# cxy1997/3D_adapt_auto_driving

Hardware: AMD Instinct MI355X
Metric: KITTI scenes/s end-to-end eval_rcnn (joint RPN+RCNN, synthetic 16384-pt scenes) (higher is better)
Workload: dtype f32; 1 GPU; BASELINE.json configs[2]: full PointRCNN RPN+RCNN inference, default.yaml shapes, random-init weights, batch=8 synthetic KITTI scenes x 16384 pts per GPU per step; scene=synth.scenes (SURVEY 8d: uniform clutter + ground + 10 dense cars), parallelism=scene-sharded x1, one final all_gather of detections, detections_gathered=652455, batch_slots=14, look_ahead=12, steps_per_launch=2

## Files before the change

3d_adapt_auto_driving_amd/_lib.py:

```python
import ctypes as C
import os

_HERE = os.path.dirname(os.path.abspath(__file__))
LIB_PATH = os.path.join(_HERE, "lib", "libprcnn_hip.so")

_P = C.c_void_p
_I = C.c_int
_F = C.c_float
_D = C.c_double
_L = C.c_longlong

class GatherProblem(C.Structure):
    _fields_ = [("b", _I), ("n", _I), ("c1", _I), ("max_tiles", C.c_long), ("P", _P), ("wxyz", _P), ("rowinfo", _P), ("rowdxyz", _P),
                ("tilecloud", _P), ("hdr", _P), ("out", _P)]


class LayerProblem(C.Structure):
    _fields_ = [("hdr", _P), ("rows", C.c_long), ("max_tiles", C.c_long), ("K", _I), ("N", _I), ("n_store", _I), ("A", _P), ("lda", C.c_long),
                ("W", _P), ("bias", _P), ("relu", _I), ("out", _P), ("ldo", C.c_long), ("b", _I), ("m", _I), ("rowinfo", _P), ("tilecloud", _P),
                ("out_col", _I), ("out_is_zero", _I)]


class SaProblem(C.Structure):
    _fields_ = [("b", _I), ("n", _I), ("m", _I), ("c3", _I), ("max_tiles", C.c_long), ("P", _P), ("wxyz", _P), ("rowinfo", _P), ("rowdxyz", _P),
# ... 21 lines not shown
    "prcnn_three_interpolate": [_I, _I, _I, _I, _P, _P, _P, _P, _P],
    "prcnn_three_interpolate_grad": [_I, _I, _I, _I, _P, _P, _P, _P, _P],
    "prcnn_query_and_group": [_I, _I, _I, _I, _F, _I, _P, _P, _P, _P, _P, _P],
    "prcnn_bias_relu_inplace": [C.c_long, _I, C.c_long, _P, _P, _P],
    "prcnn_maxpool_bias_relu": [_I, _I, _I, _I, _P, _P, _P, _P],
    "prcnn_group_cat_pm": [_I, _I, _I, _I, _I, _P, _P, _P, _P, _P, _P],
    "prcnn_gather_affine_relu_pm": [_I, _I, _I, _I, _I, _P, _P, _P, _P, _P, _P, _P],
    "prcnn_sa_mlp_fused": [_I] * 7 + [_P] * 10 + [_I, _I, _P],
    "prcnn_ball_pack": [_I, _I, _I, _I, _P, _P, _P, _P, _P, _P, _P, _P, _P],
    "prcnn_ball_pack_ex": [_I, _I, _I, _I, _I, _P, _P, _P, _P, _P, _P, _P, _P, _P, _P, _I, _P],
    "prcnn_rcnn_postprocess_blobs": [_I, _I, _I, _F, _F, _I, _I, _F, _F, _P, _F, _F, _P, _P, _P, _P, _P, _I, _P],
    "prcnn_ball_pack_groups": [_I, _I, _I, _I, _I, _P, _P, _P, _P, _P, _P, _P, _P, _P],
    "prcnn_ball_pack_rep": [_I, _I, _I, _I, _P, _P, _P, _P, _P, _P, _P, _P, _P, _P, _P],
    "prcnn_dup_rep": [_I, _I, _I, _P, _P, _P, _P, _P],
    "prcnn_rcnn_roi_geometry": [_I, _I, _I, _F, _I, _I, _F, _I] + [_P] * 9,
    "prcnn_rcnn_roi_geometry_packs": [_I, _I, _I, _F, _I, _I, _F, _I] + [_P] * 21 + [_I, _P],
    "prcnn_rows_gemm128_rows": [_L, _P, _I, _I, _P, _P, _I, _P, _P, _P, _P],
    "prcnn_sa_packed_mlp": [_I, _I, _I, _I, C.c_long] + [_P] * 11 + [_I, _I, _I, _P],
    "prcnn_packed_gather_affine": [_I, _I, _I, C.c_long] + [_P] * 7 + [_P],
    "prcnn_packed_layer": [_P, C.c_long, C.c_long, _I, _I, _I, _P, C.c_long, _P, _P, _I, _P, C.c_long, _P],
    "prcnn_split_weights_bf16x3": [_I, _I, _P, _P, _P],
    "prcnn_rows_layer_bf16x3": [C.c_long, _I, _I, _I, _P, C.c_long, _P, _P, _I, _P, C.c_long, _P],
    "prcnn_packed_layer_interp": [C.c_long, _I, _I, _P, C.c_long, _P, _P, _I, _P, C.c_long, _I, _I, _P, C.c_long, _P, _P, _P],
    "prcnn_sa_xyz_mlp_packed": [_I, _I, _I, _I, _I, C.c_long] + [_P] * 11 + [_I, _I, _I, _P],
    "prcnn_rows_dot": [C.c_long, _I, _I, _P, C.c_long, _P, _P, _P, C.c_long, _P],
    "prcnn_sa_wide_fused_supported": [_I, _I, _I],
    "prcnn_sa_wide_fused": [_I, _I, _I, _I, _I, _I, C.c_long] + [_P] * 11 + [_I, _I, _I, _P],
    "prcnn_sa_wide_fused3_supported": [_I, _I, _I, _I],
    "prcnn_sa_wide_fused3": [_I, _I, _I, _I, _I, _I, _I, C.c_long] + [_P] * 11 + [_I, _I, _I, _P],
    "prcnn_sa_packed_mlp_batch": [_I, C.POINTER(SaProblem), _P],
    "prcnn_packed_gather_affine_batch": [_I, C.POINTER(GatherProblem), _P],
    "prcnn_packed_layer_batch": [_I, C.POINTER(LayerProblem), _I, _P],
    "prcnn_rpn_tail": [_I, _I, _I] + [_P] * 7 + [_I] + [_P] * 4,
    "prcnn_rpn_tail_lin": [_I, _I, _I] + [_P] * 7 + [_I] + [_P] * 4,
    "prcnn_rpn_tail_boxes_supported": [_I, _F, _F, _I, _I],
    "prcnn_rpn_tail_lin_boxes": [_I, _I, _I] + [_P] * 7 + [_I, _F, _F, _I, _I] + [_P] * 6,
    "prcnn_selftest_fmod_two_pi": [_L, _P, _P, _P, _P],
    "prcnn_rpn_proposals_boxes": [_I, _I, _I, _I, _F, _I, _P, _P, _P, _P, _P],
    "prcnn_packed_layer_segmax": [_I, _I, C.c_long, _I, _I, _P, C.c_long, _P, _P, _P, _P, _P, _P, _I, _I, _I, _P],
    "prcnn_maxpool_pm": [C.c_long, _I, _I, _P, _P, _I, _I, _P],
    "prcnn_three_interpolate_pm": [_I, _I, _I, _I, _P, _P, _P, _P, _I, _I, _P],
    "prcnn_three_interpolate_cat_pm": [_I, _I, _I, _I, _P, _P, _P, _P, _I, _P, _P],
    "prcnn_boxes_overlap_bev": [_I, _P, _I, _P, _P, _P],
    "prcnn_boxes_iou_bev": [_I, _P, _I, _P, _P, _P],
    "prcnn_nms": [_I, _P, _P, _F, _P],
    "prcnn_nms_normal": [_I, _P, _P, _F, _P],
# ... 101 lines not shown
```

3d_adapt_auto_driving_amd/dropin/pointnet2_cuda.py:

```python
import ctypes
import importlib
import os
import sys

import torch

_pkg_dir = os.path.dirname(os.path.dirname(os.path.abspath(__file__)))
if os.path.dirname(_pkg_dir) not in sys.path:
    sys.path.insert(0, os.path.dirname(_pkg_dir))
_lib = importlib.import_module(os.path.basename(_pkg_dir) + "._lib")
IS_HIP_EXTENSION = True


def _chk(dtype, *tensors):
    for t in tensors:
        if not t.is_cuda:
            raise RuntimeError("pointnet2_cuda: tensor must be a CUDA tensor")
        if not t.is_contiguous():
            raise RuntimeError("pointnet2_cuda: tensor must be contiguous")
        if t.dtype != dtype:
            raise RuntimeError("pointnet2_cuda: expected %s, got %s" % (dtype, t.dtype))


def ball_query_wrapper(b, n, m, radius, nsample, new_xyz, xyz, idx):
# ... 441 lines not shown
        _SPLIT_W[key] = ws
    _lib.call("prcnn_rows_layer_bf16x3", R, K, N, out.size(1), a.data_ptr(), a.stride(0), ws.data_ptr(), bias.data_ptr(), int(bool(relu)),
              out.data_ptr(), out.stride(0), _lib.current_stream(a))
    return out


def packed_layer_interp_wrapper(a, wt, bias, relu, out, G, idx, weight):
    _chk(torch.float32, wt, bias, G, weight)
    _chk(torch.int32, idx)
    for t in (a, out):
        if not t.is_cuda or t.dtype != torch.float32 or t.dim() != 2 or t.stride(1) != 1:
            raise RuntimeError("pointnet2_cuda: packed_layer_interp expects 2-D float32 CUDA matrices with unit column stride")
    R, K = a.shape
    N = wt.size(1)
    B, n = idx.shape[0], idx.shape[1]
    if wt.size(0) != K or tuple(out.shape) != (R, N) or R != B * n or G.shape[0] != B or G.shape[2] != N or tuple(weight.shape) != tuple(idx.shape):
        raise RuntimeError("pointnet2_cuda: packed_layer_interp shape mismatch")
    _lib.call("prcnn_packed_layer_interp", R, K, N, a.data_ptr(), a.stride(0), wt.data_ptr(), bias.data_ptr(), int(bool(relu)),
              out.data_ptr(), out.stride(0), n, G.shape[1], G.data_ptr(), G.stride(1), idx.data_ptr(), weight.data_ptr(),
              _lib.current_stream(a))
    return out


def sa_wide_fused_supported(c1, c2, c3):
    return bool(_lib.load().prcnn_sa_wide_fused_supported(int(c1), int(c2), int(c3)))


def sa_wide_fused_wrapper(new_xyz, xyz, P, wxyz, pack, w2t, b2, w3t, b3, out, out_col, zeroed=False):
    _chk(torch.float32, new_xyz, xyz, P, wxyz, w2t, b2, w3t, b3, out)
    b, n, c1 = P.shape
    if w2t.size(0) != c1 or w3t.size(0) != w2t.size(1) or wxyz.size(1) != c1:
        raise RuntimeError("pointnet2_cuda: sa_wide_fused shape mismatch")
    _lib.call("prcnn_sa_wide_fused", b, n, new_xyz.size(1), c1, w2t.size(1), w3t.size(1), pack.max_tiles, P.data_ptr(), wxyz.data_ptr(),
              pack.rowinfo.data_ptr(), pack.rowdxyz.data_ptr(), pack.tilecloud.data_ptr(), pack.hdr.data_ptr(), w2t.data_ptr(),
              b2.data_ptr(), w3t.data_ptr(), b3.data_ptr(), out.data_ptr(), out.size(-1), out_col, int(bool(zeroed)),
              _lib.current_stream(xyz))
    return out


def sa_wide_fused3_supported(c0, c1, c2, c3):
    return bool(_lib.load().prcnn_sa_wide_fused3_supported(int(c0), int(c1), int(c2), int(c3)))


def sa_wide_fused3_wrapper(new_xyz, xyz, feats, wcat, b1, wxyz, pack, b2, b3, widths, out, out_col, zeroed=False):
    _chk(torch.float32, new_xyz, xyz, feats, wcat, b1, wxyz, b2, b3, out)
    b, n, c0 = feats.shape
# ... 213 lines not shown
```

3d_adapt_auto_driving_amd/net/fast_infer.py:

```python
import os

import torch

from ..pointnet2 import pointnet2_utils as pu
from ..pointnet2 import fused_mlp
from .._lib import has_entry
from .. import kitti_utils
from .. import roipool3d_utils
from .. import iou3d_utils


USE_ROIPOOL_CANONICAL = True
USE_RCNN_POINT_MLP = True
USE_XYZ_MLP = True
USE_PACKED = os.environ.get("PRCNN_NO_PACK") is None
USE_POOL_DEDUP = os.environ.get("PRCNN_NO_POOL_DEDUP") is None
USE_POINT_LAYER = os.environ.get("PRCNN_LIB_GEMM") is None
PAD128 = USE_PACKED and USE_POINT_LAYER
USE_RPN_TAIL = os.environ.get("PRCNN_NO_RPN_TAIL") is None
USE_SCALE_BATCH = True
USE_SA_NARROW = True
USE_WIDE_FUSED = True
EARLY_LEVELS = int(os.environ.get("PRCNN_EARLY_LEVELS", "4"))
EARLY_FP = int(os.environ.get("PRCNN_EARLY_FP", "2"))
# ... 86 lines not shown
                           % (wt.shape[0], wt.shape[1], a.shape[0]))
    if relu:
        try:
            return torch._addmm_activation(bias, a, wt)
        except (AttributeError, RuntimeError):
            return torch.addmm(bias, a, wt).relu_()
    return torch.addmm(bias, a, wt)


SPLIT_BF16 = os.environ.get("PRCNN_SPLIT_BF16") == "1"


def point_layer(a, wt, bias, relu, n_out=None):
    K, N = wt.shape
    n_out = N if n_out is None else n_out
    if (USE_PACKED and K % 128 == 0 and N % 128 == 0 and a.dim() == 2 and a.shape[1] == K and a.stride(1) == 1
            and a.stride(0) % 4 == 0 and a.data_ptr() % 16 == 0):
        out = torch.empty((a.shape[0], n_out), dtype=torch.float32, device=a.device)
        if SPLIT_BF16 and getattr(pu.pointnet2, "IS_HIP_EXTENSION", False):
            return pu.pointnet2.rows_layer_bf16x3_wrapper(a, wt, bias, relu, out)
        return pu.pointnet2.packed_layer_wrapper(a, wt, bias, relu, out)
    y = gemm_bias_act(a, wt, bias, relu)
    return y if n_out == N else y[:, :n_out].contiguous()


class _Mlp:

    def __init__(self, layers, grouped_c=None, pad128=False, in_parts=None, pad_out=False):
        self.layers = []
        self.n_out = layers[-1][0].shape[0]
        if pad128 and grouped_c is None:
            for i, (w, b, relu) in enumerate(layers):
                np_ = _round128(w.shape[0])
                if i == 0 and in_parts:
                    assert sum(in_parts) == w.shape[1]
                    wt = w.new_zeros((sum(_round128(c) for c in in_parts), np_))
                    src = dst = 0
                    for c in in_parts:
                        wt[dst:dst + c, :w.shape[0]] = w[:, src:src + c].t()
                        src, dst = src + c, dst + _round128(c)
                else:
                    wt = _pad2(w.t(), _round128(w.shape[1]), np_)
                self.layers.append((wt.contiguous(), _pad1(b, np_), relu))
            self.split = self.packed = self.wide = self.wide_cat = None
            self.padded = not pad_out
            self.narrow = None
# ... 309 lines not shown
        if not (USE_PACKED and USE_XYZ_MLP and self.sa and self.sa[0][1] and
                all(sc[3] == 0 for sc in self.sa[0][1])):
            return
        l_xyz, prev = geo["l_xyz"], None
        B = l_xyz[0].shape[0]
        for k in range(min(EARLY_LEVELS, len(self.sa))):
            npoint, scales = self.sa[k]
            lev = geo["sa"][k]
            packs = lev.get("pack") or [None] * len(scales)
            pre = bool(all(sc[2].packed is not None or sc[2].wide is not None or sc[3] == 0 for sc in scales))
            if not pre or any(pk is None for pk in packs):
                return
            width = sum(sc[2].layers[-1][0].shape[1] for sc in scales)
            oshape = (B, npoint, _round128(width) if PAD128 else width)
            out = arena.take(oshape) if arena is not None else torch.zeros(oshape, dtype=torch.float32, device=l_xyz[0].device)
            self._sa_level(scales, lev, l_xyz[k], prev, out, True)
            lev["out"] = prev = out
        if EARLY_FP > 0 and all(lev.get("out") is not None for lev in geo["sa"]) and len(geo["sa"]) == len(self.sa):
            l_feat = [None] + [lev["out"] for lev in geo["sa"]]
            geo["fp_out"] = {}
            for i in range(-1, -(min(EARLY_FP, len(self.fp) - 1) + 1), -1):
                kk = len(self.fp) + i
                idx, weight = geo["fp"][kk]
                l_feat[kk] = geo["fp_out"][kk] = self._fp_module(kk, l_feat[kk + 1], l_feat[kk], idx, weight)

    @staticmethod
    def _sa_scale(xyz, new_xyz, feats, idx, mlp, cin, out, out_col, P_pre=None, pack=None, zeroed=False, dense=False):
        ext = pu.pointnet2
        B, N, _ = xyz.shape
        M, ns = idx.shape[1], idx.shape[2]
        if USE_PACKED and mlp.packed is not None:
            wf, wx, b1, w2, b2, w3, b3 = mlp.packed
            P = P_pre if P_pre is not None else point_layer(feats.view(B * N, feats.shape[2]), wf, b1, False).view(B, N, 128)
            pk = pack if pack is not None else ext.ball_pack_wrapper(idx, xyz, new_xyz)
            ext.sa_packed_mlp_wrapper(new_xyz, xyz, P, wx, pk, w2, b2, w3, b3, out, out_col, zeroed)
            return
        if USE_PACKED and mlp.wide is not None:
            wf, wx, b1, w2, b2, w3, b3 = mlp.wide
            pk = pack if pack is not None else ext.ball_pack_wrapper(idx, xyz, new_xyz)
            if (dense and USE_WIDE_FUSED and has_entry(ext, "sa_wide_fused3_wrapper") and feats.is_contiguous() and
                    feats.shape[2] == wf.shape[0] and ext.sa_wide_fused3_supported(wf.shape[0], wf.shape[1], w2.shape[1], w3.shape[1])):
                ext.sa_wide_fused3_wrapper(new_xyz, xyz, feats, mlp.wide_cat, b1, wx, pk, b2, b3,
                                           (wf.shape[0], wf.shape[1], w2.shape[1], w3.shape[1]), out, out_col, zeroed)
                return
            P = point_layer(feats.view(B * N, feats.shape[2]), wf, b1, False).view(B, N, -1)
            if (dense and USE_WIDE_FUSED and has_entry(ext, "sa_wide_fused_wrapper") and
                    ext.sa_wide_fused_supported(wf.shape[1], w2.shape[1], w3.shape[1])):
# ... 75 lines not shown
                m0 = scales[0][2]
                if getattr(m0, "_pcat", None) is None or m0._pcat[2] is not scales[1][2].packed[0]:
                    m0._pcat = (torch.cat([sc[2].packed[0][:, :64] for sc in scales], 1).contiguous(),
                                torch.cat([sc[2].packed[2][:64] for sc in scales]).contiguous(), scales[1][2].packed[0])
                Pcat = torch.empty((B * N, 128), dtype=torch.float32, device=cur_xyz.device)
                ext.packed_layer_wrapper(flat, m0._pcat[0], m0._pcat[1], False, Pcat)
                Ps = [Pcat.view(B, N, 128)[:, :, 64 * k:64 * k + 64] for k in range(2)]
            else:
                Ps = [torch.empty((B * N, 128), dtype=torch.float32, device=cur_xyz.device) for _ in scales]
                ext.packed_layer_batch_wrapper([(flat, sc[2].packed[0], sc[2].packed[2], False, P, None) for sc, P in zip(scales, Ps)])
                Ps = [P.view(B, N, 128) for P in Ps]
            probs, col = [], 0
            for (radius, ns, mlp, cin), pack, P in zip(scales, packs, Ps):
                wf, wx, b1, w2, b2, w3, b3 = mlp.packed
                probs.append((lev["new_xyz"], cur_xyz, P, wx, pack, w2, b2, w3, b3, out, col, pre, mlp.packed_widths))
                col += mlp.layers[-1][0].shape[1]
            ext.sa_packed_mlp_batch_wrapper(probs)
        else:
            col = 0
            for (radius, ns, mlp, cin), idx, pack in zip(scales, lev["idx"], packs):
                self._sa_scale(cur_xyz, lev["new_xyz"], cur_feat, idx, mlp, cin, out, col, pack=pack, zeroed=pre)
                col += mlp.layers[-1][0].shape[1]

    def _backbone(self, xyz, geo, fuse_tail=False, feats0=None):
        l_xyz, l_feat = geo["l_xyz"], [feats0]
        B = xyz.shape[0]
        shapes, pres = [], []
        for npoint, scales in self.sa:
            width = sum(s[2].layers[-1][0].shape[1] for s in scales)
            shapes.append((B, npoint, _round128(width) if PAD128 else width))
            pres.append(bool(USE_PACKED and all(sc[2].packed is not None or sc[2].wide is not None or sc[3] == 0 for sc in scales)))
        early = [lev.get("out") if (lev.get("out") is not None and tuple(lev["out"].shape) == sh) else None for lev, sh in zip(geo["sa"], shapes)]
        sizes = [sh[0] * sh[1] * sh[2] if (pr and e is None) else 0 for sh, pr, e in zip(shapes, pres, early)]
        arena = torch.zeros((sum(sizes),), dtype=torch.float32, device=xyz.device) if sum(sizes) else None
        offs = [sum(sizes[:k]) for k in range(len(sizes))]
        for k, ((npoint, scales), lev) in enumerate(zip(self.sa, geo["sa"])):
            if early[k] is not None:
                l_feat.append(early[k])
                continue
            cur_xyz, cur_feat = l_xyz[len(l_feat) - 1], l_feat[-1]
            width = sum(s[2].layers[-1][0].shape[1] for s in scales)
            wpad = shapes[k][2]
            pre = pres[k]
            out = (arena[offs[k]:offs[k] + sizes[k]].view(shapes[k]) if pre
                   else torch.empty(shapes[k], dtype=torch.float32, device=xyz.device))
            if wpad > width and not pre:
                out[:, :, width:] = 0
            self._sa_level(scales, lev, cur_xyz, cur_feat, out, pre)
            l_feat.append(out)
        ext = pu.pointnet2
        for i in range(-1, -(len(self.fp) + 1), -1):
            k = len(self.fp) + i
            if geo.get("fp_out", {}).get(k) is not None:
                l_feat[k] = geo["fp_out"][k]
                continue
            known_feat, skip = l_feat[k + 1], l_feat[k]
            idx, weight = geo["fp"][k]
            if fuse_tail and k == 0 and self.rpn_tail is not None and skip is None and known_feat.shape[2] == 256:
                return None, (known_feat, idx, weight)
            l_feat[k] = self._fp_module(k, known_feat, skip, idx, weight)
        return (l_feat[0], None) if fuse_tail else l_feat[0]

    def _fp_module(self, k, known_feat, skip, idx, weight):
        ext = pu.pointnet2
        B, n = idx.shape[0], idx.shape[1]
        c2 = known_feat.shape[2]
        c1 = 0 if skip is None else skip.shape[2]
        mlp = self.fp[k]
        wt, b1, relu1 = mlp.layers[0]
        if (USE_FP_LINEAR and USE_POINT_LAYER and PAD128 and c1 and c1 % 128 == 0 and c2 % 128 == 0 and wt.shape[0] == c2 + c1
                and wt.shape[1] % 128 == 0 and len(mlp.layers) >= 2 and has_entry(ext, "packed_layer_interp_wrapper")):
            m = known_feat.shape[1]
            N1 = wt.shape[1]
            if getattr(self, "_zero_bias", None) is None or self._zero_bias.numel() < N1 or self._zero_bias.device != wt.device:
                self._zero_bias = torch.zeros((max(N1, 1024),), dtype=torch.float32, device=wt.device)
            G = point_layer(known_feat.view(B * m, c2), wt[:c2], self._zero_bias[:N1], False).view(B, m, N1)
            y1 = torch.empty((B * n, N1), dtype=torch.float32, device=known_feat.device)
            ext.packed_layer_interp_wrapper(skip.view(B * n, c1), wt[c2:], b1, relu1, y1, G, idx, weight)
            return mlp(y1, start=1).view(B, n, -1)
        buf = torch.empty((B, n, c2 + c1), dtype=torch.float32, device=known_feat.device)
        if c1 and c1 % 4 == 0 and c2 % 4 == 0 and has_entry(ext, "three_interpolate_cat_pm_wrapper"):
            ext.three_interpolate_cat_pm_wrapper(known_feat, idx, weight, skip, buf)
        else:
            ext.three_interpolate_pm_wrapper(known_feat, idx, weight, buf, 0)
            if c1:
                buf[:, :, c2:] = skip
        return self.fp[k](buf.view(B * n, c2 + c1)).view(B, n, -1)

    @torch.no_grad()
    def _tail_decode_cfg(self, N):
        cfg, pl = self.cfg, self.model.rpn.proposal_layer
        M = cfg[pl.mode].RPN_POST_NMS_TOP_N
        ext3 = pl_ext()
        if not (USE_FP_LINEAR and self.rpn_tail is not None and getattr(pl, "fused", False) and N <= 65536
                and cfg.TEST.RPN_DISTANCE_BASED_PROPOSE and M <= 128 and cfg.RPN.NMS_TYPE in ("normal", "rotate")
                and has_entry(pu.pointnet2, "rpn_tail_lin_boxes_wrapper") and has_entry(ext3, "rpn_proposals_boxes")
                and pu.pointnet2.rpn_tail_boxes_supported(self.rpn_tail["n_reg"], cfg.RPN.LOC_SCOPE, cfg.RPN.LOC_BIN_SIZE,
                                                         cfg.RPN.NUM_HEAD_BIN, cfg.RPN.LOC_XZ_FINE)):
            return None
        return (cfg.RPN.LOC_SCOPE, cfg.RPN.LOC_BIN_SIZE, cfg.RPN.NUM_HEAD_BIN, cfg.RPN.LOC_XZ_FINE, pl._anchor)

    def rpn_stage(self, pts_input, geo=None, want_reg=False):
        cfg = self.cfg
        self.check_weights()
        if pts_input.shape[-1] != 3 + self.in_feat:
            raise ValueError("pts_input has %d channels, the backbone was built for 3 + %d" % (pts_input.shape[-1], self.in_feat))
        feats0 = None
        if self.in_feat:
            xyz = pts_input[..., 0:3].contiguous()
            feats0 = pts_input.new_zeros((pts_input.shape[0], pts_input.shape[1], _round128(self.in_feat) if PAD128 else self.in_feat))
            feats0[..., :self.in_feat] = pts_input[..., 3:]
        else:
            xyz = pts_input.contiguous()
        if geo is None:
            geo = self.geometry(xyz)
        B, N, _ = xyz.shape
        with self._strictly():
            feats, tail = self._backbone(xyz, geo, fuse_tail=True, feats0=feats0)
        if tail is not None:
            known_feat, idx, weight = tail
            tw = self.rpn_tail
            feats = torch.empty((B, N, 128), dtype=torch.float32, device=xyz.device)
            rpn_cls = torch.empty((B, N, 1), dtype=torch.float32, device=xyz.device)
            dec = None if want_reg or self.in_feat else self._tail_decode_cfg(N)
            rpn_reg = torch.empty((B, N, tw["n_reg"]), dtype=torch.float32, device=xyz.device) if dec is None else None
            rpn_boxes = None
            if USE_FP_LINEAR and has_entry(pu.pointnet2, "rpn_tail_lin_wrapper"):
                m = known_feat.shape[1]
                G = point_layer(known_feat.view(B * m, known_feat.shape[2]), tw["w1"], tw["zero128"], False).view(B, m, 128)
                if dec is not None:
                    rpn_boxes = torch.empty((B, N, 7), dtype=torch.float32, device=xyz.device)
                    pu.pointnet2.rpn_tail_lin_boxes_wrapper(G, idx, weight, tw["wcat_lin"], tw["bcat"], tw["wc2"], tw["bc2"], tw["n_reg"],
                                                            dec[0], dec[1], dec[2], dec[3], dec[4], xyz, feats, rpn_cls, rpn_boxes)
                else:
                    pu.pointnet2.rpn_tail_lin_wrapper(G, idx, weight, tw["wcat_lin"], tw["bcat"], tw["wc2"], tw["bc2"], feats, rpn_cls, rpn_reg)
            else:
                pu.pointnet2.rpn_tail_wrapper(known_feat, idx, weight, tw["wcat"], tw["bcat"], tw["wc2"], tw["bc2"], feats, rpn_cls, rpn_reg)
        else:
            flat = feats.view(B * N, -1)
            rpn_cls = self.rpn_cls(flat).view(B, N, -1)
            rpn_reg = self.rpn_reg(flat).view(B, N, -1)
            if feats.shape[2] != self.fp[0].n_out:
                feats = feats[:, :, :self.fp[0].n_out].contiguous()
            rpn_boxes = None
        out = {"rpn_cls": rpn_cls, "rpn_reg": rpn_reg, "rpn_boxes": rpn_boxes, "backbone_xyz": xyz, "rpn_features": feats, "groups": geo.get("groups")}
        out["rpn_scores_raw"] = rpn_cls[:, :, 0].contiguous()
        return out

    @torch.no_grad()
    def point_aux(self, st):
        if "seg_result" not in st:
            ext = pu.pointnet2
# ... 306 lines not shown
```

include/prcnn_hip.h:

```cpp
#ifndef PRCNN_HIP_H
#define PRCNN_HIP_H

#ifdef __cplusplus
extern "C" {
#endif

#define PRCNN_OK 0
#define PRCNN_EINVAL (-1)
#define PRCNN_ELAUNCH (-2)

int prcnn_version(void);
const char *prcnn_last_error(void);
int prcnn_opt_n_threads(int work_size);


int prcnn_ball_query(int b, int n, int m, float radius, int nsample,
                     const float *new_xyz, const float *xyz, int *idx, void *stream);

int prcnn_ball_query_full(int b, int n, int m, float radius, int nsample, const float *new_xyz, const float *xyz, int *idx,
                          void *stream);

int prcnn_set_ball_query_mode(int mode);

int prcnn_group_points(int b, int c, int n, int npoints, int nsample,
// ... 99 lines not shown
    const float *bias; int relu; float *out; long ldo;
    int b, m; const unsigned int *rowinfo; const int *tilecloud; int out_col, out_is_zero;
} prcnn_layer_problem;
typedef struct prcnn_sa_problem {
    int b, n, m, c3; long max_tiles; const float *P; const float *wxyz; const unsigned int *rowinfo; const float *rowdxyz;
    const int *tilecloud; const unsigned int *hdr; const float *w2t; const float *b2; const float *w3t; const float *b3;
    float *out; int out_stride, out_col, out_is_zero;
    int c1, c2;
} prcnn_sa_problem;
int prcnn_sa_packed_mlp_batch(int nprob, const prcnn_sa_problem *problems, void *stream);
int prcnn_packed_gather_affine_batch(int nprob, const prcnn_gather_problem *problems, void *stream);
int prcnn_packed_layer_batch(int nprob, const prcnn_layer_problem *problems, int segmax, void *stream);
int prcnn_packed_gather_affine(int b, int n, int c1, long max_tiles, const float *P, const float *wxyz,
                               const unsigned int *rowinfo, const float *rowdxyz, const int *tilecloud,
                               const unsigned int *hdr, float *out, void *stream);
int prcnn_packed_layer(const unsigned int *hdr, long rows, long max_tiles, int K, int N, int n_store, const float *A,
                       long lda, const float *W, const float *bias, int relu, float *out, long ldo, void *stream);
int prcnn_split_weights_bf16x3(int K, int N, const float *W, void *out, void *stream);
int prcnn_rows_layer_bf16x3(long rows, int K, int N, int n_store, const float *A, long lda, const void *wsplit, const float *bias,
                            int relu, float *out, long ldo, void *stream);
int prcnn_packed_layer_interp(long rows, int K, int N, const float *A, long lda, const float *W, const float *bias, int relu,
                              float *out, long ldo, int n_per_cloud, int m_known, const float *G, long ldg, const int *idx,
                              const float *weight, void *stream);
int prcnn_sa_xyz_mlp_packed(int b, int m, int c1, int c2, int c3, long max_tiles, const unsigned int *rowinfo,
                            const float *rowdxyz, const int *tilecloud, const unsigned int *hdr, const float *w1,
                            const float *b1, const float *w2, const float *b2, const float *w3, const float *b3,
                            float *out, int out_stride, int out_col, int out_is_zero, void *stream);
int prcnn_rows_dot(long rows, int K, int n, const float *A, long lda, const float *W, const float *bias, float *out,
                   long ldo, void *stream);
int prcnn_rpn_tail(int b, int n, int m, const float *known, const int *idx, const float *weight, const float *wcat,
                   const float *bcat, const float *wc2, const float *bc2, int n_reg, float *feats, float *cls, float *reg,
                   void *stream);
int prcnn_rpn_tail_lin(int b, int n, int m, const float *G, const int *idx, const float *weight, const float *wcat,
                       const float *bcat, const float *wc2, const float *bc2, int n_reg, float *feats, float *cls,
                       float *reg, void *stream);
int prcnn_rpn_tail_boxes_supported(int channels, float loc_scope, float loc_bin_size, int num_head_bin, int xz_fine);
int prcnn_selftest_fmod_two_pi(long n, const float *a, float *out_mine, float *out_lib, void *stream);
int prcnn_rpn_tail_lin_boxes(int b, int n, int m, const float *G, const int *idx, const float *weight, const float *wcat,
                             const float *bcat, const float *wc2, const float *bc2, int n_reg, float loc_scope, float loc_bin_size,
                             int num_head_bin, int xz_fine, const float *anchor_size_host, const float *xyz, float *feats,
                             float *cls, float *boxes, void *stream);
int prcnn_packed_layer_segmax(int b, int m, long max_tiles, int K, int N, const float *A, long lda, const float *W,
                              const float *bias, const unsigned int *rowinfo, const int *tilecloud,
                              const unsigned int *hdr, float *out, int out_stride, int out_col, int out_is_zero, void *stream);

int prcnn_rcnn_point_mlp(long r, int ld, int fcol, const float *rows, const float *wu1, const float *bu1,
// ... 141 lines not shown
```

profiles/mfma_launch_shapes.py:

```python
import collections
import csv
import os
import sys

rows = list(csv.DictReader(open(sys.argv[1])))
rows.sort(key=lambda r: int(r["Start_Timestamp"]))
half = rows[len(rows) // 2:]
steps = max(1, int(os.environ.get("PRCNN_PAIR", "2")) * sum(1 for r in half if "rpn_tail" in r["Kernel_Name"]))
by = collections.defaultdict(lambda: [0, 0.0])
for r in half:
    name = r["Kernel_Name"]
    if not any(k in name for k in ("packed_layer", "sa_packed", "sa_wide", "rcnn_entrance", "rpn_tail", "rcnn_point")):
        continue
    key = (name.replace("void ", "").replace("prcnn::", "").split("(")[0][:44], r.get("Stream_Id", "?"),
           "%sx%sx%s" % (r["Grid_Size_X"], r["Grid_Size_Y"], r["Grid_Size_Z"]), r["Workgroup_Size_X"])
    by[key][0] += 1
    by[key][1] += (int(r["End_Timestamp"]) - int(r["Start_Timestamp"])) / 1e3
print("second half of the trace = %d steps\n\n| kernel | stream | grid (threads) | wg | launches per step | avg us | us per step |\n|---|---|---|---|---|---|---|" % steps)
for k, v in sorted(by.items(), key=lambda kv: -kv[1][1]):
    print("| `%s` | %s | %s | %s | %.2f | %.1f | %.1f |" % (k[0], k[1], k[2], k[3], v[0] / steps, v[1] / v[0], v[1] / steps))
```

Measured before the change: 8653 scenes/s.

## Fuse FP second layer with next level's coarse projection in one chain kernel

Adds an MFMA kernel that computes a FP module's second layer (bias+ReLU) and immediately multiplies the result, kept in LDS, by the next FP module's coarse-feature weight slice (or the RPN tail's first weight). The next level then receives the precomputed product instead of running a separate point_layer GEMM on the coarse features. This removes one kernel launch and one write and re-read of the intermediate activation per FP level. The kernel uses a persistent ticket-based tile scheduler with software-pipelined weight and activation prefetch. It only applies when dimensions are multiples of 128 and the intermediate fits in LDS.

```diff
diff --git a/3d_adapt_auto_driving_amd/_lib.py b/3d_adapt_auto_driving_amd/_lib.py
--- a/3d_adapt_auto_driving_amd/_lib.py
+++ b/3d_adapt_auto_driving_amd/_lib.py
@@ -67,6 +67,8 @@
     "prcnn_split_weights_bf16x3": [_I, _I, _P, _P, _P],
     "prcnn_rows_layer_bf16x3": [C.c_long, _I, _I, _I, _P, C.c_long, _P, _P, _I, _P, C.c_long, _P],
     "prcnn_packed_layer_interp": [C.c_long, _I, _I, _P, C.c_long, _P, _P, _I, _P, C.c_long, _I, _I, _P, C.c_long, _P, _P, _P],
+    "prcnn_packed_layer_chain2_supported": [_I, _I, _I],
+    "prcnn_packed_layer_chain2": [C.c_long, _I, _I, _I, _P, C.c_long, _P, _P, _P, _P, C.c_long, _P],
     "prcnn_sa_xyz_mlp_packed": [_I, _I, _I, _I, _I, C.c_long] + [_P] * 11 + [_I, _I, _I, _P],
     "prcnn_rows_dot": [C.c_long, _I, _I, _P, C.c_long, _P, _P, _P, C.c_long, _P],
     "prcnn_sa_wide_fused_supported": [_I, _I, _I],
diff --git a/3d_adapt_auto_driving_amd/csrc/fp_chain.hip b/3d_adapt_auto_driving_amd/csrc/fp_chain.hip
--- /dev/null
+++ b/3d_adapt_auto_driving_amd/csrc/fp_chain.hip
@@ -0,0 +1,243 @@
+#include "common.hpp"
+#include "segmax.hpp"
+
+namespace prcnn {
+
+unsigned int *next_ticket(hipStream_t st);
+
+typedef float f32x4 __attribute__((ext_vector_type(4)));
+constexpr int FC_LD = 128 + 4;
+constexpr size_t FC_LDS_MAX = 160 * 1024;
+
+#define FC_VM_DRAIN __builtin_amdgcn_s_waitcnt(0x0F70);
+#define FC_SADD(x, y) asm volatile("s_add_u32 %0, %0, %1" : "+s"(x) : "s"(y) : "scc");
+
+struct FcLane { int j, h, r0, chunk; };
+
+template <int R, bool PW, bool PA>
+__device__ __forceinline__ void fc_stage(const float *T, float *TN, const float (&wf)[64], float (&wn)[64], f32x16 &acc0, f32x16 &acc1,
+                                         const __amdgpu_buffer_rsrc_t wrs, const unsigned int loff, unsigned int wo,
+                                         const unsigned int row_bytes, const __amdgpu_buffer_rsrc_t ars, const unsigned int a_lane,
+                                         unsigned int ao, const unsigned int a_row_bytes, const FcLane &L)
+{
+    constexpr int NA = R / 8;
+    const float *a0p = T + L.j * FC_LD + 64 * L.h, *a1p = T + (32 + L.j) * FC_LD + 64 * L.h;
+    f32x4 a0 = *reinterpret_cast<const f32x4 *>(a0p);
+    f32x4 a1 = a0;
+    if constexpr (R == 64) a1 = *reinterpret_cast<const f32x4 *>(a1p);
+    f32x4 ar[NA];
+    const unsigned int a8 = 8u * a_row_bytes;
+#pragma unroll
+    for (int g = 0; g < 16; ++g) {
+        f32x4 n0 = a0, n1 = a1;
+        if (g < 15) {
+            n0 = *reinterpret_cast<const f32x4 *>(a0p + 4 * (g + 1));
+            if constexpr (R == 64) n1 = *reinterpret_cast<const f32x4 *>(a1p + 4 * (g + 1));
+        }
+        __builtin_amdgcn_sched_barrier(0);
+        acc0 = __builtin_amdgcn_mfma_f32_32x32x2f32(a0.x, wf[4 * g + 0], acc0, 0, 0, 0);
+        if constexpr (R == 64) acc1 = __builtin_amdgcn_mfma_f32_32x32x2f32(a1.x, wf[4 * g + 0], acc1, 0, 0, 0);
+        if constexpr (PA) {
+            if (g < NA) {
+                ar[g] = __builtin_bit_cast(f32x4, __builtin_amdgcn_raw_buffer_load_b128(ars, a_lane, ao, 0));
+                FC_SADD(ao, a8)
+            } else if (g >= 8 && g < 8 + NA) {
+                *reinterpret_cast<f32x4 *>(TN + (L.r0 + 8 * (g - 8)) * FC_LD + 4 * L.chunk) = ar[g - 8];
+            }
+        }
+        if constexpr (PW) {
+#pragma unroll
+            for (int q = 0; q < 6; ++q)
+                if (6 * g + q < 64) {
+                    wn[6 * g + q] = __uint_as_float(__builtin_amdgcn_raw_buffer_load_b32(wrs, loff, wo, 0));
+                    FC_SADD(wo, row_bytes)
+                }
+        }
+        __builtin_amdgcn_sched_barrier(0);
+        acc0 = __builtin_amdgcn_mfma_f32_32x32x2f32(a0.y, wf[4 * g + 1], acc0, 0, 0, 0);
+        if constexpr (R == 64) acc1 = __builtin_amdgcn_mfma_f32_32x32x2f32(a1.y, wf[4 * g + 1], acc1, 0, 0, 0);
+        acc0 = __builtin_amdgcn_mfma_f32_32x32x2f32(a0.z, wf[4 * g + 2], acc0, 0, 0, 0);
+        if constexpr (R == 64) acc1 = __builtin_amdgcn_mfma_f32_32x32x2f32(a1.z, wf[4 * g + 2], acc1, 0, 0, 0);
+        acc0 = __builtin_amdgcn_mfma_f32_32x32x2f32(a0.w, wf[4 * g + 3], acc0, 0, 0, 0);
+        if constexpr (R == 64) acc1 = __builtin_amdgcn_mfma_f32_32x32x2f32(a1.w, wf[4 * g + 3], acc1, 0, 0, 0);
+        a0 = n0; a1 = n1;
+    }
+}
+
+template <int R>
+__global__ __launch_bounds__(256, R == 64 ? 1 : 2) void fp_chain_kernel(long rows, int K, int N2, int N3, const float *__restrict__ A, long lda,
+                                                          const float *__restrict__ W2, const float *__restrict__ b2,
+                                                          const float *__restrict__ W3, float *__restrict__ out, long ldo,
+                                                          unsigned int *__restrict__ ticket)
+{
+    extern __shared__ float fc_lds[];
+    __shared__ unsigned int s_item[2];
+    constexpr int TILE = R * FC_LD;
+    float *At = fc_lds, *Yt = fc_lds + 2 * TILE;
+    const int tid = threadIdx.x, lane = tid & 63;
+    const FcLane L = {lane & 31, lane >> 5, tid >> 5, tid & 31};
+    const int w = __builtin_amdgcn_readfirstlane(tid >> 6);
+    const int np2 = K >> 7, nc2 = N2 >> 7, nc3 = N3 >> 7;
+    const unsigned int n_tiles = (unsigned int)((rows + R - 1) / R);
+    const __amdgpu_buffer_rsrc_t w2rs = __builtin_amdgcn_make_buffer_rsrc((void *)W2, 0, K * N2 * 4, 0x00020000);
+    const __amdgpu_buffer_rsrc_t w3rs = __builtin_amdgcn_make_buffer_rsrc((void *)W3, 0, N2 * N3 * 4, 0x00020000);
+    const unsigned int rb2 = (unsigned int)N2 * 4u, rb3 = (unsigned int)N3 * 4u;
+    const unsigned int a_row_bytes = (unsigned int)lda * 4u, o_row_bytes = (unsigned int)ldo * 4u;
+    const unsigned int a_lane = (unsigned int)L.r0 * a_row_bytes + 16u * L.chunk;
+    const unsigned int col = (unsigned int)(32 * w + L.j);
+    const unsigned int loff2 = ((unsigned int)(64 * L.h) * (unsigned int)N2 + col) * 4u;
+    const unsigned int loff3 = ((unsigned int)(64 * L.h) * (unsigned int)N3 + col) * 4u;
+    auto tile_rsrc = [&](unsigned int t) __attribute__((always_inline)) {
+        const long left = rows - (long)t * R;
+        return __builtin_amdgcn_make_buffer_rsrc((void *)(A + (long)t * R * lda), 0, (int)((left < R ? left : R) * (long)a_row_bytes), 0x00020000);
+    };
+    unsigned int t = blockIdx.x;
+    __amdgpu_buffer_rsrc_t ars = tile_rsrc(t);
+    float wa[64], wb[64];
+    {
+#pragma unroll
+        for (int s = 0; s < 64; ++s)
+            wa[s] = __uint_as_float(__builtin_amdgcn_raw_buffer_load_b32(w2rs, loff2, (unsigned int)s * rb2, 0));
+#pragma unroll
+        for (int i = 0; i < R / 8; ++i)
+            *reinterpret_cast<f32x4 *>(At + (L.r0 + 8 * i) * FC_LD + 4 * L.chunk) =
+                __builtin_bit_cast(f32x4, __builtin_amdgcn_raw_buffer_load_b128(ars, a_lane, (unsigned int)(8 * i) * a_row_bytes, 0));
+    }
+    int pp = 0;
+    int slot = 0;
+    FC_VM_DRAIN
+    while (true) {
+        unsigned int drawn = 0, next = 0xffffffffu;
+        for (int cb = 0; cb < nc2; ++cb) {
+            f32x16 acc0 = {0}, acc1 = {0};
+            const float bcol = b2[cb * 128 + (int)col];
+            for (int p = 0; p < np2; ++p) {
+                lds_barrier();
+                if (cb == 0 && p == 0 && tid == 0) drawn = gridDim.x + atomicAdd(ticket, 1u);
+                const float *T = At + (pp & 1) * TILE;
+                float *TN = At + ((pp + 1) & 1) * TILE;
+                if (p + 1 < np2 || cb + 1 < nc2) {
+                    const int pn = p + 1 < np2 ? p + 1 : 0, cbn = p + 1 < np2 ? cb : cb + 1;
+                    fc_stage<R, true, true>(T, TN, wa, wb, acc0, acc1, w2rs, loff2 + 512u * cbn, (unsigned int)(pn * 128) * rb2, rb2, ars,
+                                            a_lane, (unsigned int)(pn * 128) * 4u, a_row_bytes, L);
+                    ++pp;
+                } else {
+                    fc_stage<R, true, false>(T, TN, wa, wb, acc0, acc1, w3rs, loff3, 0u, rb3, ars, a_lane, 0u, a_row_bytes, L);
+                }
+#pragma unroll
+                for (int s = 0; s < 64; ++s) wa[s] = wb[s];
+                FC_VM_DRAIN
+            }
+            float *Y = Yt + cb * TILE;
+#pragma unroll
+            for (int r = 0; r < 16; ++r) {
+                const int row = (r & 3) + 8 * (r >> 2) + 4 * L.h;
+                Y[row * FC_LD + (int)col] = fmaxf(acc0[r] + bcol, 0.f);
+                if constexpr (R == 64) Y[(32 + row) * FC_LD + (int)col] = fmaxf(acc1[r] + bcol, 0.f);
+            }
+        }
+        if (tid == 0) s_item[slot] = drawn;
+        for (int cb = 0; cb < nc3; ++cb) {
+            f32x16 acc0 = {0}, acc1 = {0};
+            for (int p = 0; p < nc2; ++p) {
+                lds_barrier();
+                const float *T = Yt + p * TILE;
+                float *TN = At + ((pp + 1) & 1) * TILE;
+                if (p + 1 < nc2 || cb + 1 < nc3) {
+                    const int pn = p + 1 < nc2 ? p + 1 : 0, cbn = p + 1 < nc2 ? cb : cb + 1;
+                    fc_stage<R, true, false>(T, TN, wa, wb, acc0, acc1, w3rs, loff3 + 512u * cbn, (unsigned int)(pn * 128) * rb3, rb3, ars,
+                                             a_lane, 0u, a_row_bytes, L);
+                } else {
+                    next = s_item[slot];
+                    if (next < n_tiles) {
+                        const __amdgpu_buffer_rsrc_t ars_n = tile_rsrc(next);
+                        fc_stage<R, true, true>(T, TN, wa, wb, acc0, acc1, w2rs, loff2, 0u, rb2, ars_n, a_lane, 0u, a_row_bytes, L);
+                        ++pp;
+                    } else {
+                        fc_stage<R, false, false>(T, TN, wa, wb, acc0, acc1, w3rs, loff3, 0u, rb3, ars, a_lane, 0u, a_row_bytes, L);
+                    }
+                }
+                if (next >= n_tiles && p + 1 == nc2 && cb + 1 == nc3) break;
+#pragma unroll
+                for (int s = 0; s < 64; ++s) wa[s] = wb[s];
+                FC_VM_DRAIN
+            }
+            const long left = rows - (long)t * R;
+            const __amdgpu_buffer_rsrc_t ors = __builtin_amdgcn_make_buffer_rsrc(
+                (void *)(out + (long)t * R * ldo), 0, (int)((left < R ? left : R) * (long)o_row_bytes), 0x00020000);
+            const unsigned int o_lane = (unsigned int)(4 * L.h) * o_row_bytes + ((unsigned int)cb * 128u + col) * 4u;
+#pragma unroll
+            for (int r = 0; r < 16; ++r) {
+                const unsigned int so = (unsigned int)((r & 3) + 8 * (r >> 2)) * o_row_bytes;
+                __builtin_amdgcn_raw_buffer_store_b32(__float_as_uint(__fadd_rn(acc0[r], 0.f)), ors, o_lane, so, 0);
+                if constexpr (R == 64)
+                    __builtin_amdgcn_raw_buffer_store_b32(__float_as_uint(__fadd_rn(acc1[r], 0.f)), ors, o_lane, so + 32u * o_row_bytes, 0);
+            }
+        }
+        if (next >= n_tiles) break;
+        t = next;
+        ars = tile_rsrc(t);
+        slot ^= 1;
+    }
+    if (tid == 0) ticket_release(ticket);
+}
+
+static int fc_cus()
+{
+    static const int n = [] {
+        int v = 0;
+        if (hipDeviceGetAttribute(&v, hipDeviceAttributeMultiprocessorCount, current_device()) != hipSuccess || v <= 0) { (void)hipGetLastError(); v = 256; }
+        return v;
+    }();
+    return n;
+}
+
+static int fc_tile_rows(int N2)
+{
+    const size_t tiles = 2 + (size_t)(N2 / 128);
+    if (tiles * 64 * FC_LD * sizeof(float) + 64 <= FC_LDS_MAX) return 64;
+    if (tiles * 32 * FC_LD * sizeof(float) + 64 <= FC_LDS_MAX) return 32;
+    return 0;
+}
+
+}
+
+using namespace prcnn;
+
+extern "C" int prcnn_packed_layer_chain2_supported(int K, int N2, int N3)
+{
+    return K > 0 && N2 > 0 && N3 > 0 && K % 128 == 0 && N2 % 128 == 0 && N3 % 128 == 0 && fc_tile_rows(N2) == 64;
+}
+
+extern "C" int prcnn_packed_layer_chain2(long rows, int K, int N2, int N3, const float *A, long lda, const float *W2, const float *b2,
+                                         const float *W3, float *out, long ldo, void *stream)
+{
+    PRCNN_REQUIRE(rows >= 0 && K > 0 && N2 > 0 && N3 > 0 && K % 128 == 0 && N2 % 128 == 0 && N3 % 128 == 0,
+                  "packed_layer_chain2: K=%d, N2=%d, N3=%d must be multiples of 128", K, N2, N3);
+    PRCNN_REQUIRE(lda >= K && lda % 4 == 0 && ldo >= N3, "packed_layer_chain2: bad leading dimensions");
+    const int R = fc_tile_rows(N2);
+    PRCNN_REQUIRE(R > 0, "packed_layer_chain2: an intermediate of %d columns does not fit LDS", N2);
+    PRCNN_REQUIRE((long)K * N2 * 4 < (1L << 31) && (long)N2 * N3 * 4 < (1L << 31) && 64 * lda * 4 < (1L << 31) && 64 * ldo * 4 < (1L << 31),
+                  "packed_layer_chain2: matrix too large for a buffer resource");
+    if (rows == 0) return PRCNN_OK;
+    PRCNN_REQUIRE(A && W2 && b2 && W3 && out, "packed_layer_chain2: null pointer");
+    PRCNN_REQUIRE(((uintptr_t)A & 15) == 0 && (((uintptr_t)W2 | (uintptr_t)W3 | (uintptr_t)out | (uintptr_t)b2) & 3) == 0,
+                  "packed_layer_chain2: 16-byte aligned rows of A required");
+    const long tiles = (rows + R - 1) / R;
+    PRCNN_REQUIRE(tiles < 0x7fffffffL - 4096, "packed_layer_chain2: too many rows");
+    hipStream_t st = (hipStream_t)stream;
+    const size_t lds = (2 + (size_t)(N2 / 128)) * R * FC_LD * sizeof(float);
+    const void *kern = R == 64 ? (const void *)fp_chain_kernel<64> : (const void *)fp_chain_kernel<32>;
+    const int rc = ensure_dynamic_lds(kern, lds, "packed_layer_chain2");
+    if (rc != PRCNN_OK) return rc;
+    const long per_cu = (long)(FC_LDS_MAX / (lds + 64)) < 2 ? (long)(FC_LDS_MAX / (lds + 64)) : 2;
+    const long cap = (long)fc_cus() * per_cu;
+    unsigned int *ticket = next_ticket(st);
+    if (!ticket) { set_error("packed_layer_chain2: cannot set up the tile ticket"); return PRCNN_ELAUNCH; }
+    const dim3 grid((unsigned)(tiles < cap ? tiles : cap));
+    if (R == 64)
+        hipLaunchKernelGGL(fp_chain_kernel<64>, grid, dim3(256), lds, st, rows, K, N2, N3, A, lda, W2, b2, W3, out, ldo, ticket);
+    else
+        hipLaunchKernelGGL(fp_chain_kernel<32>, grid, dim3(256), lds, st, rows, K, N2, N3, A, lda, W2, b2, W3, out, ldo, ticket);
+    return check_launch("packed_layer_chain2");
+}
diff --git a/3d_adapt_auto_driving_amd/dropin/pointnet2_cuda.py b/3d_adapt_auto_driving_amd/dropin/pointnet2_cuda.py
--- a/3d_adapt_auto_driving_amd/dropin/pointnet2_cuda.py
+++ b/3d_adapt_auto_driving_amd/dropin/pointnet2_cuda.py
@@ -487,6 +487,24 @@
     return out
 
 
+def packed_layer_chain2_supported(K, N2, N3):
+    return bool(_lib.call("prcnn_packed_layer_chain2_supported", int(K), int(N2), int(N3)))
+
+
+def packed_layer_chain2_wrapper(a, w2, b2, w3, out):
+    _chk(torch.float32, w2, b2, w3)
+    for t in (a, out):
+        if not t.is_cuda or t.dtype != torch.float32 or t.dim() != 2 or t.stride(1) != 1:
+            raise RuntimeError("pointnet2_cuda: packed_layer_chain2 expects 2-D float32 CUDA matrices with unit column stride")
+    R, K = a.shape
+    N2, N3 = w2.size(1), w3.size(1)
+    if w2.size(0) != K or w3.size(0) != N2 or b2.numel() != N2 or tuple(out.shape) != (R, N3):
+        raise RuntimeError("pointnet2_cuda: packed_layer_chain2 shape mismatch")
+    _lib.call("prcnn_packed_layer_chain2", R, K, N2, N3, a.data_ptr(), a.stride(0), w2.data_ptr(), b2.data_ptr(), w3.data_ptr(),
+              out.data_ptr(), out.stride(0), _lib.current_stream(a))
+    return out
+
+
 def sa_wide_fused_supported(c1, c2, c3):
     return bool(_lib.load().prcnn_sa_wide_fused_supported(int(c1), int(c2), int(c3)))
 
diff --git a/3d_adapt_auto_driving_amd/net/fast_infer.py b/3d_adapt_auto_driving_amd/net/fast_infer.py
--- a/3d_adapt_auto_driving_amd/net/fast_infer.py
+++ b/3d_adapt_auto_driving_amd/net/fast_infer.py
@@ -132,6 +132,15 @@
         return pu.pointnet2.packed_layer_wrapper(a, wt, bias, relu, out)
     y = gemm_bias_act(a, wt, bias, relu)
     return y if n_out == N else y[:, :n_out].contiguous()
+
+
+class _ReadyG:
+
+    def __init__(self, G):
+        self.G = G
+
+    def __getitem__(self, sl):
+        return _ReadyG(self.G[sl])
 
 
 class _Mlp:
@@ -487,7 +496,8 @@
             for i in range(-1, -(min(EARLY_FP, len(self.fp) - 1) + 1), -1):
                 kk = len(self.fp) + i
                 idx, weight = geo["fp"][kk]
-                l_feat[kk] = geo["fp_out"][kk] = self._fp_module(kk, l_feat[kk + 1], l_feat[kk], idx, weight)
+                next_w = self._next_coarse(kk, l_feat, False, False) if kk >= 2 else None
+                l_feat[kk] = geo["fp_out"][kk] = self._fp_module(kk, l_feat[kk + 1], l_feat[kk], idx, weight, next_w=next_w)
 
     @staticmethod
     def _sa_scale(xyz, new_xyz, feats, idx, mlp, cin, out, out_col, P_pre=None, pack=None, zeroed=False, dense=False):
@@ -609,7 +619,7 @@
                 self._sa_scale(cur_xyz, lev["new_xyz"], cur_feat, idx, mlp, cin, out, col, pack=pack, zeroed=pre)
                 col += mlp.layers[-1][0].shape[1]
 
-    def _backbone(self, xyz, geo, fuse_tail=False, feats0=None):
+    def _backbone(self, xyz, geo, fuse_tail=False, feats0=None, tail_product=False):
         l_xyz, l_feat = geo["l_xyz"], [feats0]
         B = xyz.shape[0]
         shapes, pres = [], []
@@ -643,27 +653,60 @@
                 continue
             known_feat, skip = l_feat[k + 1], l_feat[k]
             idx, weight = geo["fp"][k]
-            if fuse_tail and k == 0 and self.rpn_tail is not None and skip is None and known_feat.shape[2] == 256:
+            if (fuse_tail and k == 0 and self.rpn_tail is not None and skip is None and
+                    (isinstance(known_feat, _ReadyG) or known_feat.shape[2] == 256)):
                 return None, (known_feat, idx, weight)
-            l_feat[k] = self._fp_module(k, known_feat, skip, idx, weight)
+            l_feat[k] = self._fp_module(k, known_feat, skip, idx, weight, next_w=self._next_coarse(k, l_feat, fuse_tail, tail_product))
         return (l_feat[0], None) if fuse_tail else l_feat[0]
 
-    def _fp_module(self, k, known_feat, skip, idx, weight):
+    def _fp_coarse_weights(self, k, c2, skip):
+        c1 = 0 if skip is None else skip.shape[2]
+        mlp = self.fp[k]
+        wt = mlp.layers[0][0]
+        if (USE_FP_LINEAR and USE_POINT_LAYER and PAD128 and c1 and c1 % 128 == 0 and c2 % 128 == 0 and wt.shape[0] == c2 + c1
+                and wt.shape[1] % 128 == 0 and len(mlp.layers) >= 2 and has_entry(pu.pointnet2, "packed_layer_interp_wrapper")):
+            return wt[:c2]
+        return None
+
+    def _next_coarse(self, k, l_feat, fuse_tail, tail_product):
+        if k == 0:
+            return None
+        n2 = self.fp[k].layers[-1][0].shape[1]
+        if k == 1 and fuse_tail and self.rpn_tail is not None and l_feat[0] is None and n2 == 256:
+            if tail_product and USE_FP_LINEAR and has_entry(pu.pointnet2, "rpn_tail_lin_wrapper"):
+                return self.rpn_tail["w1"]
+            return None
+        return self._fp_coarse_weights(k - 1, n2, l_feat[k - 1])
+
+    def _fp_module(self, k, known_feat, skip, idx, weight, next_w=None):
         ext = pu.pointnet2
         B, n = idx.shape[0], idx.shape[1]
-        c2 = known_feat.shape[2]
         c1 = 0 if skip is None else skip.shape[2]
         mlp = self.fp[k]
         wt, b1, relu1 = mlp.layers[0]
-        if (USE_FP_LINEAR and USE_POINT_LAYER and PAD128 and c1 and c1 % 128 == 0 and c2 % 128 == 0 and wt.shape[0] == c2 + c1
-                and wt.shape[1] % 128 == 0 and len(mlp.layers) >= 2 and has_entry(ext, "packed_layer_interp_wrapper")):
-            m = known_feat.shape[1]
+        ready = known_feat if isinstance(known_feat, _ReadyG) else None
+        c2 = wt.shape[0] - c1 if ready is not None else known_feat.shape[2]
+        w_coarse = self._fp_coarse_weights(k, c2, skip)
+        if ready is not None and (w_coarse is None or ready.G.shape[2] != wt.shape[1]):
+            raise RuntimeError("FastPointRCNN: FP module %d was handed a coarse product but does not run in its product form" % k)
+        if w_coarse is not None:
             N1 = wt.shape[1]
-            if getattr(self, "_zero_bias", None) is None or self._zero_bias.numel() < N1 or self._zero_bias.device != wt.device:
-                self._zero_bias = torch.zeros((max(N1, 1024),), dtype=torch.float32, device=wt.device)
-            G = point_layer(known_feat.view(B * m, c2), wt[:c2], self._zero_bias[:N1], False).view(B, m, N1)
-            y1 = torch.empty((B * n, N1), dtype=torch.float32, device=known_feat.device)
+            if ready is not None:
+                G = ready.G
+            else:
+                m = known_feat.shape[1]
+                if getattr(self, "_zero_bias", None) is None or self._zero_bias.numel() < N1 or self._zero_bias.device != wt.device:
+                    self._zero_bias = torch.zeros((max(N1, 1024),), dtype=torch.float32, device=wt.device)
+                G = point_layer(known_feat.view(B * m, c2), w_coarse, self._zero_bias[:N1], False).view(B, m, N1)
+            y1 = torch.empty((B * n, N1), dtype=torch.float32, device=G.device)
             ext.packed_layer_interp_wrapper(skip.view(B * n, c1), wt[c2:], b1, relu1, y1, G, idx, weight)
+            if next_w is not None and len(mlp.layers) == 2 and not mlp.padded and not SPLIT_BF16 and USE_PACKED:
+                w2, b2, relu2 = mlp.layers[1]
+                if (relu2 and w2.shape[1] == next_w.shape[0] and next_w.is_contiguous() and has_entry(ext, "packed_layer_chain2_wrapper")
+                        and ext.packed_layer_chain2_supported(w2.shape[0], w2.shape[1], next_w.shape[1])):
+                    Gn = torch.empty((B * n, next_w.shape[1]), dtype=torch.float32, device=G.device)
+                    ext.packed_layer_chain2_wrapper(y1, w2, b2, next_w, Gn)
+                    return _ReadyG(Gn.view(B, n, -1))
             return mlp(y1, start=1).view(B, n, -1)
         buf = torch.empty((B, n, c2 + c1), dtype=torch.float32, device=known_feat.device)
         if c1 and c1 % 4 == 0 and c2 % 4 == 0 and has_entry(ext, "three_interpolate_cat_pm_wrapper"):
@@ -703,7 +746,7 @@
             geo = self.geometry(xyz)
         B, N, _ = xyz.shape
         with self._strictly():
-            feats, tail = self._backbone(xyz, geo, fuse_tail=True, feats0=feats0)
+            feats, tail = self._backbone(xyz, geo, fuse_tail=True, feats0=feats0, tail_product=True)
         if tail is not None:
             known_feat, idx, weight = tail
             tw = self.rpn_tail
@@ -713,8 +756,11 @@
             rpn_reg = torch.empty((B, N, tw["n_reg"]), dtype=torch.float32, device=xyz.device) if dec is None else None
             rpn_boxes = None
             if USE_FP_LINEAR and has_entry(pu.pointnet2, "rpn_tail_lin_wrapper"):
-                m = known_feat.shape[1]
-                G = point_layer(known_feat.view(B * m, known_feat.shape[2]), tw["w1"], tw["zero128"], False).view(B, m, 128)
+                if isinstance(known_feat, _ReadyG):
+                    G = known_feat.G
+                else:
+                    m = known_feat.shape[1]
+                    G = point_layer(known_feat.view(B * m, known_feat.shape[2]), tw["w1"], tw["zero128"], False).view(B, m, 128)
                 if dec is not None:
                     rpn_boxes = torch.empty((B, N, 7), dtype=torch.float32, device=xyz.device)
                     pu.pointnet2.rpn_tail_lin_boxes_wrapper(G, idx, weight, tw["wcat_lin"], tw["bcat"], tw["wc2"], tw["bc2"], tw["n_reg"],
diff --git a/include/prcnn_hip.h b/include/prcnn_hip.h
--- a/include/prcnn_hip.h
+++ b/include/prcnn_hip.h
@@ -145,6 +145,9 @@
 int prcnn_packed_layer_interp(long rows, int K, int N, const float *A, long lda, const float *W, const float *bias, int relu,
                               float *out, long ldo, int n_per_cloud, int m_known, const float *G, long ldg, const int *idx,
                               const float *weight, void *stream);
+int prcnn_packed_layer_chain2_supported(int K, int N2, int N3);
+int prcnn_packed_layer_chain2(long rows, int K, int N2, int N3, const float *A, long lda, const float *W2, const float *b2,
+                              const float *W3, float *out, long ldo, void *stream);
 int prcnn_sa_xyz_mlp_packed(int b, int m, int c1, int c2, int c3, long max_tiles, const unsigned int *rowinfo,
                             const float *rowdxyz, const int *tilecloud, const unsigned int *hdr, const float *w1,
                             const float *b1, const float *w2, const float *b2, const float *w3, const float *b3,
diff --git a/profiles/mfma_launch_shapes.py b/profiles/mfma_launch_shapes.py
--- a/profiles/mfma_launch_shapes.py
+++ b/profiles/mfma_launch_shapes.py
@@ -10,7 +10,7 @@
 by = collections.defaultdict(lambda: [0, 0.0])
 for r in half:
     name = r["Kernel_Name"]
-    if not any(k in name for k in ("packed_layer", "sa_packed", "sa_wide", "rcnn_entrance", "rpn_tail", "rcnn_point")):
+    if not any(k in name for k in ("packed_layer", "fp_chain", "sa_packed", "sa_wide", "rcnn_entrance", "rpn_tail", "rcnn_point")):
         continue
     key = (name.replace("void ", "").replace("prcnn::", "").split("(")[0][:44], r.get("Stream_Id", "?"),
            "%sx%sx%s" % (r["Grid_Size_X"], r["Grid_Size_Y"], r["Grid_Size_Z"]), r["Workgroup_Size_X"])
```

Result: no change. 8585 scenes/s (-0.8%).
